# TheRealOrange/icer_compression

Hardware: AMD Instinct MI355X
Metric: Mpixels/s encode (bit-exact), 4096x4096 gray (higher is better)
Workload: dtype int16

## Files before the change

### icer_compression_amd/csrc/coder_core.hpp

```cpp
#pragma once
#include "events.hpp"
#include "icer_tables.hpp"
#include "wave.hpp"

#if defined(ICER_ISA_MARKERS) && !defined(ICER_WAVE_EMU)
#define ICER_STR2(x) #x
#define ICER_STR(x) ICER_STR2(x)
#define ICER_MARK(what) asm volatile("; ICER_MARK " what " line " ICER_STR(__LINE__));
#else
#define ICER_MARK(what)
#endif

#if defined(ICER_WAVE_EMU) && defined(ICER_WAVE_THREADS)
#include <assert.h>
#include <atomic>
#include <thread>
#define ICER_EMU_COUNT(i)
#define ICER_LOAD_CNT(x) __atomic_load_n(&(x), __ATOMIC_ACQUIRE)
#define ICER_POLL_PAUSE(n) std::this_thread::yield()
#define ICER_SET_ABORT2() __atomic_store_n(&s.abort, 2u, __ATOMIC_RELAXED)
#define ICER_FENCE_ACQ() std::atomic_thread_fence(std::memory_order_acquire)
#define ICER_FENCE_REL() std::atomic_thread_fence(std::memory_order_release)
#define ICER_STORE_CNT(x, v) __atomic_store_n(&(x), (v), __ATOMIC_RELEASE)
#define ICER_LANE0
// ... 311 lines not shown
                {                                                                                     \
                    if (PRED) {                                                                       \
                        LV(TOUT) = t0_ + (uint32_t)mbcnt64(m_, lane);                                 \
                        LV(ZOUT) = z0_ + (uint32_t)mbcnt64(zm_, lane);                                \
                    }                                                                                 \
                }                                                                                     \
                FOR_LANES { if ((uint32_t)lane == (C)) { LV(ctot) = t0_ + n_; LV(czer) = z0_ + nz_; } }      \
            } else {                                                                                  \
                const uint32_t kc_ = kRescaleCap - 1 - t0_;   \
                const int lc_ = ffs64(BALLOT((PRED) && (uint32_t)mbcnt64(m_, lane) == kc_));          \
                const uint32_t zc_ = (uint32_t)popc64(zm_ & ((2ull << lc_) - 1ull));                  \
                const uint32_t zat_ = z0_ + zc_;                                                      \
                const uint32_t zr_ = (zat_ > kRescaleCap / 2) ? (zat_ >> 1) : zat_;                   \
                FOR_LANES                                                                             \
                {                                                                                     \
                    if (PRED) {                                                                       \
                        const uint32_t rk_ = (uint32_t)mbcnt64(m_, lane), zb_ = (uint32_t)mbcnt64(zm_, lane); \
                        if (rk_ <= kc_) { LV(TOUT) = t0_ + rk_; LV(ZOUT) = z0_ + zb_; }               \
                        else { LV(TOUT) = kRescaleCap / 2 + (rk_ - kc_ - 1); LV(ZOUT) = zr_ + (zb_ - zc_); } \
                    }                                                                                 \
                }                                                                                     \
                FOR_LANES { if ((uint32_t)lane == (C)) { LV(ctot) = kRescaleCap / 2 + (n_ - kc_ - 1); LV(czer) = zr_ + (nz_ - zc_); } } \
            }                                                                                         \
        }                                                                                             \
    }

ICER_DEV bool flush_stage(CoderShared &s, const UnitArgs &a, bool final_partial)
{
    DECL_LANE;
    const uint32_t bp = s.bitpos;
    const uint32_t first = s.flushed_words;
    uint32_t last = bp >> 5;
    if (final_partial && (bp & 31u)) last++;
    const bool fits = last <= a.cap_words;
    const uint32_t stop = fits ? last : a.cap_words;
    FOR_LANES
    {
        for (uint32_t wi = first + (uint32_t)lane; wi < last; wi += 64) {
            const uint32_t v = s.stage[wi & (kStageWords - 1)];
            if (wi < stop) a.out_words[wi] = v;
            s.stage[wi & (kStageWords - 1)] = 0;
        }
    }
    WAVE_SYNC();
    FOR_LANES
    {
        if (lane == 0) s.flushed_words = last;
    }
    WAVE_SYNC();
    return fits && (bp >> 3) < a.cap_words * 4u;
}

ICER_DEV uint64_t below64(uint32_t x) { return x >= 64u ? ~0ull : ((1ull << x) - 1ull); }
ICER_DEV uint32_t own_bit(uint64_t A, int lane) { return ((lane < 32 ? (uint32_t)A : (uint32_t)(A >> 32)) >> (lane & 31)) & 1u; }
ICER_DEV uint64_t lanes_below(int lane)
{
    const uint32_t lo = lane < 32 ? (1u << (lane & 31)) - 1u : ~0u, hi = lane < 32 ? 0u : (1u << (lane & 31)) - 1u;
    return (uint64_t)lo | ((uint64_t)hi << 32);
}
ICER_DEV uint32_t cnt_lt(uint64_t A1, uint64_t A2, uint32_t pos)
{
    return (uint32_t)(popc64(A1 & below64((pos + 1u) >> 1)) + popc64(A2 & below64(pos >> 1)));
}
ICER_DEV uint32_t cnt_lt_own(uint64_t A1, uint64_t A2, int lane, uint32_t slot)
{
    return (uint32_t)(mbcnt64(A1, lane) + mbcnt64(A2, lane)) + (slot ? own_bit(A1, lane) : 0u);
}
ICER_DEV int last_le(uint64_t A1, uint64_t A2, uint32_t pos)
{
    const uint64_t c1 = A1 & below64((pos >> 1) + 1u), c2 = A2 & below64((pos + 1u) >> 1);
    const int k1 = c1 ? 2 * (63 - clz64(c1)) : -1, k2 = c2 ? 2 * (63 - clz64(c2)) + 1 : -1;
    return k1 > k2 ? k1 : k2;
}
ICER_DEV int last_lt(uint64_t A1, uint64_t A2, uint32_t pos) { return pos == 0u ? -1 : last_le(A1, A2, pos - 1u); }
ICER_DEV int last_lt_own(uint64_t A1, uint64_t A2, int lane, uint32_t slot)
{
    const uint64_t lt = lanes_below(lane);
    const uint64_t c1 = A1 & (slot ? (lt << 1) | 1ull : lt), c2 = A2 & lt;
    const int k1 = c1 ? 2 * (63 - clz64(c1)) : -1, k2 = c2 ? 2 * (63 - clz64(c2)) + 1 : -1;
    return k1 > k2 ? k1 : k2;
}
ICER_DEV int last_le_own(uint64_t A1, uint64_t A2, int lane, uint32_t slot)
{
    const uint64_t lt = lanes_below(lane), le = (lt << 1) | 1ull;
    const uint64_t c1 = A1 & le, c2 = A2 & (slot ? le : lt);
    const int k1 = c1 ? 2 * (63 - clz64(c1)) : -1, k2 = c2 ? 2 * (63 - clz64(c2)) + 1 : -1;
    return k1 > k2 ? k1 : k2;
}
ICER_DEV uint32_t cnt_lt1(uint64_t A1, uint32_t pos) { return (uint32_t)popc64(A1 & below64((pos + 1u) >> 1)); }
ICER_DEV uint32_t cnt_lt_own1(uint64_t A1, int lane, uint32_t slot) { return (uint32_t)mbcnt64(A1, lane) + (slot ? own_bit(A1, lane) : 0u); }
ICER_DEV int last_lt_own1(uint64_t A1, int lane, uint32_t slot)
{
    const uint64_t lt = lanes_below(lane);
    const uint64_t c1 = A1 & (slot ? (lt << 1) | 1ull : lt);
    return c1 ? 2 * (63 - clz64(c1)) : -1;
}
ICER_DEV int last_le_own1(uint64_t A1, int lane)
{
    const uint64_t c1 = A1 & ((lanes_below(lane) << 1) | 1ull);
    return c1 ? 2 * (63 - clz64(c1)) : -1;
}

ICER_DEV uint32_t wave_drain(CoderShared &s, uint32_t limit, uint32_t max_rounds)
{
    DECL_LANE;
    const uint32_t popped0 = s.popped;
    uint32_t head = popped0 & (kRingWords - 1), used = limit - popped0, bitpos = s.bitpos;
    uint32_t npop = 0;
    for (uint32_t round = 0; round < max_rounds; round++) {
        LANEVAR(uint32_t, w); LANEVAR(uint32_t, len); LANEVAR(uint32_t, off);
        FOR_LANES
        {
            LV(w) = (uint32_t)lane < used ? RING_LD((head + (uint32_t)lane) & (kRingWords - 1)) : 0u;
        }
        const uint64_t done = BALLOT((LV(w) & kWordDone) != 0u);
        const uint32_t n = (uint32_t)ffs64(~done);
        if (n == 0) break;
        FOR_LANES
        {
            LV(len) = (uint32_t)lane < n ? ((LV(w) >> 11) & 15u) : 0u;
        }
        const uint64_t L0 = BALLOT(LV(len) & 1u), L1 = BALLOT(LV(len) & 2u), L2 = BALLOT(LV(len) & 4u), L3 = BALLOT(LV(len) & 8u);
        const uint32_t total = (uint32_t)(popc64(L0) + 2 * popc64(L1) + 4 * popc64(L2) + 8 * popc64(L3));
        FOR_LANES
        {
            LV(off) = (uint32_t)(mbcnt64(L0, lane) + 2 * mbcnt64(L1, lane) + 4 * mbcnt64(L2, lane) + 8 * mbcnt64(L3, lane));
        }
        FOR_LANES
        {
            if (LV(len)) {
                const uint32_t p = bitpos + LV(off), wi = (p >> 5) & (kStageWords - 1), sh = p & 31u;
                const uint32_t code = LV(w) & 0x3FFu;
                LDS_OR(s.stage[wi], code << sh);
                if (sh + LV(len) > 32u) LDS_OR(s.stage[(wi + 1) & (kStageWords - 1)], code >> (32u - sh));
            }
        }
        bitpos += total;
        head = (head + n) & (kRingWords - 1);
        used -= n;
        npop += n;
        if (n < 64u) break;
    }
    WAVE_SYNC();
    FOR_LANES
    {
        if (lane == 0) s.bitpos = bitpos;
    }
    ICER_PUBLISH(s.popped, popped0 + npop)
    WAVE_SYNC();
    return npop;
}


struct PixelWave {
    LANEVAR(uint32_t, nb);
    uint32_t fetched = ~0u;
    uint64_t blank = 0;
    uint32_t blank_base = ~0u;
};

#define ICER_BLANK_MASK(J)                                                                             \
    if (((J) & ~63u) != cw.blank_base) {                                                               \
        cw.blank_base = (J) & ~63u;                                                                    \
        cw.blank = BALLOT(cw.blank_base + (uint32_t)lane < nchunks && (uint32_t)a.sig[cw.blank_base + (uint32_t)lane] <= lsb); \
    }
#define ICER_IS_BLANK(J) (((cw.blank >> ((J) & 63u)) & 1ull) != 0ull)

#define ICER_UNPACK_EVENT_BYTE(B, V1, C1, B1, V2, C2, B2)                                              \
    {                                                                                                  \
        const uint32_t b_ = (B), c4_ = b_ & 15u;                                                       \
        V1 = c4_ != kEvNone ? 1u : 0u;                                                                 \
        C1 = c4_ == kEvUncoded ? 31u : c4_;                                                            \
        B1 = (b_ >> 4) & 1u;                                                                           \
        V2 = (c4_ <= 8u && (b_ & 16u)) ? 1u : 0u;        \
        C2 = 12u + ((b_ >> 5) & 3u);                                                                   \
        B2 = (b_ >> 7) & 1u;                                                                           \
    }

ICER_DEV void pixel_wave_run(CoderShared &s, const UnitArgs &a, PixelWave &cw, uint32_t j0, uint32_t j1, uint32_t k, uint32_t npw)
{
    DECL_LANE;
    ICER_TIMERS_DECL
    const uint32_t nchunks = (a.w * a.h + 63u) / 64u;
    const uint32_t lsb = (uint32_t)a.lsb;
    const uint32_t jfirst = j0 + (k + npw - j0 % npw) % npw;
    if (cw.fetched != jfirst && jfirst < nchunks) {
        ICER_BLANK_MASK(jfirst)
        if (!ICER_IS_BLANK(jfirst)) { FOR_LANES { LV(cw.nb) = a.ev[(size_t)jfirst * 64u + (uint32_t)lane]; } }
        cw.fetched = jfirst;
    }

    for (uint32_t j = jfirst; j < j1; j += npw) {
        LANEVAR(uint32_t, valid1); LANEVAR(uint32_t, ctx1); LANEVAR(uint32_t, bit1);
        LANEVAR(uint32_t, valid2); LANEVAR(uint32_t, ctx2); LANEVAR(uint32_t, bit2);
        ICER_BLANK_MASK(j)
        const bool blank = ICER_IS_BLANK(j);
        LANEVAR(uint32_t, eb);
        FOR_LANES { LV(eb) = blank ? 0u : LV(cw.nb); }
        if (j + npw < nchunks) {
            ICER_BLANK_MASK(j + npw)
            if (!ICER_IS_BLANK(j + npw)) { FOR_LANES { LV(cw.nb) = a.ev[(size_t)(j + npw) * 64u + (uint32_t)lane]; } }
        }
        cw.fetched = j + npw;
        FOR_LANES { ICER_UNPACK_EVENT_BYTE(LV(eb), LV(valid1), LV(ctx1), LV(bit1), LV(valid2), LV(ctx2), LV(bit2)) }
        LANEVAR(uint32_t, w1); LANEVAR(uint32_t, w2); LANEVAR(uint32_t, cnw);
#define ICER_MATCH(KEY, V, B0, B1, B2, B3) \
        ((V) & (((KEY)&1u) ? (B0) : ~(B0)) & (((KEY)&2u) ? (B1) : ~(B1)) & (((KEY)&4u) ? (B2) : ~(B2)) & (((KEY)&8u) ? (B3) : ~(B3)))
#ifdef ICER_WAVE_EMU
        assert(blank == (BALLOT(!LV(valid1) || LV(ctx1) != 0u || LV(bit1) != 0u || LV(valid2)) == 0ull));
#endif
        if (blank) {
            FOR_LANES
            {
                LV(w1) = 0x80u | ((uint32_t)lane << 8) | ((uint32_t)lane << 16);
                LV(w2) = 0;
                LV(cnw) = lane == 0 ? (64u | (64u << 8)) : 0u;
            }
        } else {
            const uint64_t V = BALLOT(LV(valid1) && LV(ctx1) != 31u);
            const uint64_t B0 = BALLOT(LV(ctx1) & 1u), B1 = BALLOT(LV(ctx1) & 2u), B2 = BALLOT(LV(ctx1) & 4u), B3 = BALLOT(LV(ctx1) & 8u);
            const uint64_t ZM = BALLOT(LV(bit1) == 0u);
            const uint64_t U = BALLOT(LV(valid2) != 0u);
            const uint64_t C0 = BALLOT((LV(ctx2) - 12u) & 1u), C1 = BALLOT((LV(ctx2) - 12u) & 2u), C2 = BALLOT((LV(ctx2) - 12u) & 4u);
            const uint64_t ZN = BALLOT(LV(bit2) == 0u);
            LANEVAR(uint32_t, om_lo); LANEVAR(uint32_t, om_hi); LANEVAR(uint32_t, g1l); LANEVAR(uint32_t, g1h); LANEVAR(uint32_t, g2l); LANEVAR(uint32_t, g2h);
            LANEVAR(uint32_t, x1); LANEVAR(uint32_t, x2);
            FOR_LANES
            {
                uint64_t m = 0, zs = ZM;
                if (U) {
                    const bool sg = lane >= 12;
                    const uint32_t key = sg ? (uint32_t)lane - 12u : (uint32_t)lane;
                    const uint64_t vv = sg ? U : V, b0 = sg ? C0 : B0, b1 = sg ? C1 : B1, b2 = sg ? C2 : B2, b3 = sg ? 0ull : B3;
                    if (lane <= 16) m = ICER_MATCH(key, vv, b0, b1, b2, b3);
                    zs = sg ? ZN : ZM;
                } else if (lane < 12) m = ICER_MATCH((uint32_t)lane, V, B0, B1, B2, B3);
                LV(om_lo) = (uint32_t)m; LV(om_hi) = (uint32_t)(m >> 32);
                LV(cnw) = (uint32_t)popc64(m) | ((uint32_t)popc64(m & zs) << 8);
                LV(x1) = LV(ctx1) & 31u; LV(x2) = LV(ctx2) & 31u;
                LV(g1l) = 0; LV(g1h) = 0; LV(g2l) = 0; LV(g2h) = 0;
            }
            WAVE_GATHER(g1l, om_lo, x1) WAVE_GATHER(g1h, om_hi, x1)
            if (U) { WAVE_GATHER(g2l, om_lo, x2) WAVE_GATHER(g2h, om_hi, x2) }
            FOR_LANES
            {
                LV(w1) = 0; LV(w2) = 0;
                if (LV(valid1)) {
                    LV(w1) = 0x80u | (LV(bit1) << 5) | LV(ctx1);
                    if (LV(ctx1) != 31u) {
                        const uint64_t m = (uint64_t)LV(g1l) | ((uint64_t)LV(g1h) << 32);
                        LV(w1) |= ((uint32_t)mbcnt64(m, lane) << 8) | ((uint32_t)mbcnt64(m & ZM, lane) << 16);
                    }
                }
                if (LV(valid2)) {
                    LV(w2) = 0x80u | (LV(bit2) << 5) | LV(ctx2);
                    const uint64_t m = (uint64_t)LV(g2l) | ((uint64_t)LV(g2h) << 32);
                    LV(w2) |= ((uint32_t)mbcnt64(m, lane) << 8) | ((uint32_t)mbcnt64(m & ZN, lane) << 16);
                }
            }
        }
#undef ICER_MATCH
        ICER_TICK(0)
        ICER_WAIT_CNT(s.a_done, ad_, j < ad_ + kQueueDepth, ab_, ICER_BP_SLEEP)
        if (ab_) break;
        ICER_TICK(1)
        PixelSlot &o = s.pq[j % kQueueDepth];
        FOR_LANES
        {
            o.e[lane][0] = LV(w1);
            o.e[lane][1] = LV(w2);
            if (lane < 17) o.cn[lane] = (uint16_t)LV(cnw);
            if (lane == 17) o.cn[17] = blank ? 1u : 0u;
        }
        ICER_PUBLISH(s.p_done[k], j + 1u)
    }
    ICER_TIMERS_STORE(a.timers)
}

struct CountWave {
    LANEVAR(uint32_t, czer);
    LANEVAR(uint32_t, ctot);
};

ICER_DEV void count_wave_run(CoderShared &s, const UnitArgs &a, CountWave &cs, uint32_t j0, uint32_t j1, uint32_t npw)
{
    DECL_LANE;
    ICER_TIMERS_DECL
    LANEVAR(uint32_t, czer); LANEVAR(uint32_t, ctot);
    FOR_LANES
    {
        LV(czer) = j0 == 0 ? 2u : LV(cs.czer);
        LV(ctot) = j0 == 0 ? 4u : LV(cs.ctot);
    }
    for (uint32_t j = j0; j < j1; j++) {
        ICER_WAIT_CNT(s.p_done[j % npw], pd_, pd_ > j, ab_, 1)
        if (ab_) break;
        ICER_TICK(2)
        const PixelSlot &in = s.pq[j % kQueueDepth];
        LANEVAR(uint32_t, valid1); LANEVAR(uint32_t, ctx1); LANEVAR(uint32_t, bit1);
        LANEVAR(uint32_t, valid2); LANEVAR(uint32_t, ctx2); LANEVAR(uint32_t, bit2);
        LANEVAR(uint32_t, z1); LANEVAR(uint32_t, t1); LANEVAR(uint32_t, z2); LANEVAR(uint32_t, t2);
        LANEVAR(uint32_t, rk1); LANEVAR(uint32_t, zb1); LANEVAR(uint32_t, rk2); LANEVAR(uint32_t, zb2);
        LANEVAR(uint32_t, cn); LANEVAR(uint32_t, cnz);
        FOR_LANES
        {
            const uint32_t c1 = in.e[lane][0], c2 = in.e[lane][1];
            LV(valid1) = (c1 >> 7) & 1u; LV(ctx1) = c1 & 31u; LV(bit1) = (c1 >> 5) & 1u; LV(rk1) = (c1 >> 8) & 255u; LV(zb1) = (c1 >> 16) & 255u;
            LV(valid2) = (c2 >> 7) & 1u; LV(ctx2) = c2 & 31u; LV(bit2) = (c2 >> 5) & 1u; LV(rk2) = (c2 >> 8) & 255u; LV(zb2) = (c2 >> 16) & 255u;
            const uint32_t w = lane < 17 ? (uint32_t)in.cn[lane] : 0u;
            LV(cn) = w & 255u; LV(cnz) = w >> 8;
            LV(z1) = 1; LV(t1) = 2;
            LV(z2) = 0; LV(t2) = 0;
        }

#ifdef ICER_WAVE_THREADS
        assert(ICER_LOAD_CNT(s.p_done[j % npw]) <= j + kQueueDepth);
#endif
        {
            LANEVAR(uint32_t, t0); LANEVAR(uint32_t, zz0); LANEVAR(uint32_t, idx);
            FOR_LANES { LV(idx) = LV(ctx1) & 15u; }
            WAVE_GATHER(t0, ctot, idx)
            WAVE_GATHER(zz0, czer, idx)
            FOR_LANES
            {
                if (LV(valid1) && LV(ctx1) != 31u) { LV(t1) = LV(t0) + LV(rk1); LV(z1) = LV(zz0) + LV(zb1); }
                LV(idx) = LV(ctx2);
            }
            if (BALLOT(LV(valid2) != 0u)) {
                WAVE_GATHER(t0, ctot, idx)
                WAVE_GATHER(zz0, czer, idx)
            }
            LANEVAR(uint32_t, cross);
            FOR_LANES
            {
                if (LV(valid2)) { LV(t2) = LV(t0) + LV(rk2); LV(z2) = LV(zz0) + LV(zb2); }
                LV(cross) = 0;
                if (lane < 17) {
                    if (LV(ctot) + LV(cn) < kRescaleCap) { LV(ctot) += LV(cn); LV(czer) += LV(cnz); }
                    else LV(cross) = 1;
                }
            }
            for (uint64_t rem = BALLOT(LV(cross) != 0u); rem; rem &= rem - 1ull) {
                const uint32_t c = (uint32_t)ffs64(rem);
                if (c < 12u) ICER_CTX_STEP(c, LV(valid1) && LV(ctx1) == c, LV(bit1) == 0u, z1, t1)
                else ICER_CTX_STEP(c, LV(valid2) && LV(ctx2) == c, LV(bit2) == 0u, z2, t2)
            }
        }
        ICER_TICK(3)

        LANEVAR(uint32_t, ev1); LANEVAR(uint32_t, ev2);
        FOR_LANES
        {
            uint32_t e1 = 0, e2 = 0;
            if (LV(valid1)) {
                uint32_t z = LV(z1), t = LV(t1), b = LV(bit1);
                if (z < (t >> 1)) { z = t - z; b ^= 1u; }
                e1 = 0x80u | (b << 5) | pick_bin(s.tab.binlut, z, t);
            }
            if (LV(valid2)) {
                uint32_t z = LV(z2), t = LV(t2), b = LV(bit2);
                if (z < (t >> 1)) { z = t - z; b ^= 1u; }
                e2 = 0x80u | (b << 5) | pick_bin(s.tab.binlut, z, t);
            }
            LV(ev1) = e1;
            LV(ev2) = e2;
        }
        ICER_TICK(4)
        ICER_WAIT_CNT(s.b_done, bd_, j < bd_ + kQueueDepth, ab2_, ICER_BP_SLEEP)
        if (ab2_) break;
        ICER_TICK(5)
        EventSlot &q = s.eq[j % kQueueDepth];
        FOR_LANES
        {
            q.ev1[lane] = (uint8_t)LV(ev1);
            q.ev2[lane] = (uint8_t)LV(ev2);
            if (lane == 0) q.blank = in.cn[17];
            if (lane < kNumBins) q.cnt[lane] = LV(czer) | (LV(ctot) << 16);
        }
        ICER_PUBLISH(s.a_done, j + 1u)
    }
    FOR_LANES { LV(cs.czer) = LV(czer); LV(cs.ctot) = LV(ctot); }
    ICER_TIMERS_STORE(a.timers)
}

constexpr uint32_t kPrefixRing = 32;
struct PrefixRing {
    uint16_t cn[kPrefixRing][20];
    uint8_t ev[kPrefixRing][64];
};
static_assert(sizeof(PrefixRing) <= sizeof(EventSlot) * kQueueDepth, "the prefix ring lies over the event queue");
ICER_DEV PrefixRing &prefix_ring(CoderShared &s) { return *reinterpret_cast<PrefixRing *>(&s.eq[0]); }

ICER_DEV void pixel_prefix_run(CoderShared &s, const UnitArgs &a, PixelWave &cw, uint32_t j0, uint32_t j1, uint32_t k, uint32_t npw)
{
    DECL_LANE;
    PrefixRing &ring = prefix_ring(s);
    const uint32_t nchunks = (a.w * a.h + 63u) / 64u;
    const uint32_t lsb = (uint32_t)a.lsb;
    const uint32_t jfirst = j0 + (k + npw - j0 % npw) % npw;
    if (cw.fetched != jfirst && jfirst < nchunks) {
        ICER_BLANK_MASK(jfirst)
        if (!ICER_IS_BLANK(jfirst)) { FOR_LANES { LV(cw.nb) = a.ev[(size_t)jfirst * 64u + (uint32_t)lane]; } }
        cw.fetched = jfirst;
    }
    for (uint32_t j = jfirst; j < j1; j += npw) {
        ICER_BLANK_MASK(j)
        const bool blank = ICER_IS_BLANK(j);
        LANEVAR(uint32_t, eb); LANEVAR(uint32_t, cnw);
        FOR_LANES { LV(eb) = blank ? 0u : LV(cw.nb); }
        if (j + npw < nchunks) {
            ICER_BLANK_MASK(j + npw)
            if (!ICER_IS_BLANK(j + npw)) { FOR_LANES { LV(cw.nb) = a.ev[(size_t)(j + npw) * 64u + (uint32_t)lane]; } }
        }
        cw.fetched = j + npw;
        if (blank) {
            FOR_LANES { LV(cnw) = lane == 0 ? (64u | (64u << 8)) : 0u; }
        } else {
            LANEVAR(uint32_t, valid1); LANEVAR(uint32_t, ctx1); LANEVAR(uint32_t, bit1);
            LANEVAR(uint32_t, valid2); LANEVAR(uint32_t, ctx2); LANEVAR(uint32_t, bit2);
            FOR_LANES { ICER_UNPACK_EVENT_BYTE(LV(eb), LV(valid1), LV(ctx1), LV(bit1), LV(valid2), LV(ctx2), LV(bit2)) }
#define ICER_MATCH(KEY, V, B0, B1, B2, B3) \
            ((V) & (((KEY)&1u) ? (B0) : ~(B0)) & (((KEY)&2u) ? (B1) : ~(B1)) & (((KEY)&4u) ? (B2) : ~(B2)) & (((KEY)&8u) ? (B3) : ~(B3)))
            const uint64_t V = BALLOT(LV(valid1) && LV(ctx1) != 31u);
            const uint64_t B0 = BALLOT(LV(ctx1) & 1u), B1 = BALLOT(LV(ctx1) & 2u), B2 = BALLOT(LV(ctx1) & 4u), B3 = BALLOT(LV(ctx1) & 8u);
            const uint64_t ZM = BALLOT(LV(bit1) == 0u);
            const uint64_t U = BALLOT(LV(valid2) != 0u);
            const uint64_t C0 = BALLOT((LV(ctx2) - 12u) & 1u), C1 = BALLOT((LV(ctx2) - 12u) & 2u), C2 = BALLOT((LV(ctx2) - 12u) & 4u);
            const uint64_t ZN = BALLOT(LV(bit2) == 0u);
            FOR_LANES
            {
                const bool sg = lane >= 12;
                const uint32_t key = sg ? (uint32_t)lane - 12u : (uint32_t)lane;
                const uint64_t vv = sg ? U : V, b0 = sg ? C0 : B0, b1 = sg ? C1 : B1, b2 = sg ? C2 : B2, b3 = sg ? 0ull : B3;
                const uint64_t m = lane <= 16 ? ICER_MATCH(key, vv, b0, b1, b2, b3) : 0ull;
                LV(cnw) = (uint32_t)popc64(m) | ((uint32_t)popc64(m & (sg ? ZN : ZM)) << 8);
            }
#undef ICER_MATCH
        }
        ICER_WAIT_CNT(s.a_done, ad_, j < ad_ + kPrefixRing, ab_, 2)
        if (ab_) break;
        FOR_LANES
        {
            if (lane < 17) ring.cn[j % kPrefixRing][lane] = (uint16_t)LV(cnw);
            ring.ev[j % kPrefixRing][lane] = (uint8_t)LV(eb);
        }
        ICER_PUBLISH(s.p_done[k], j + 1u)
    }
}

ICER_DEV uint32_t prefix_frontier(CoderShared &s, uint32_t npw)
{
    DECL_LANE;
    LANEVAR(uint32_t, nxt);
    FOR_LANES
    {
        const uint32_t pd = (uint32_t)lane < npw ? ICER_LOAD_CNT(s.p_done[lane]) : 0u;
        LV(nxt) = (uint32_t)lane < npw ? ~(pd ? pd - 1u + npw : (uint32_t)lane) : 0u;
    }
    uint32_t m;
    WAVE_MAX(m, nxt)
    return ~m;
}

ICER_DEV void count_prefix_run(CoderShared &s, const UnitArgs &a, CountWave &cs, uint32_t j0, uint32_t j1, uint32_t npw)
{
    DECL_LANE;
    (void)a;
    PrefixRing &ring = prefix_ring(s);
    LANEVAR(uint32_t, czer); LANEVAR(uint32_t, ctot);
    FOR_LANES
    {
        LV(czer) = j0 == 0 ? 2u : LV(cs.czer);
        LV(ctot) = j0 == 0 ? 4u : LV(cs.ctot);
    }
    uint32_t avail = j0;
    for (uint32_t j = j0; j < j1; j++) {
        if (j >= avail) {
            avail = prefix_frontier(s, npw);
            if (avail <= j) {
                ICER_PUBLISH(s.a_done, j)
                ICER_WAIT_UNTIL((avail = prefix_frontier(s, npw)) > j || ICER_LOAD_CNT(s.abort))
            }
            if (ICER_LOAD_CNT(s.abort)) break;
            ICER_ACQUIRE()
        }
        LANEVAR(uint32_t, cross);
        FOR_LANES
        {
            const uint32_t w = lane < 17 ? (uint32_t)ring.cn[j % kPrefixRing][lane] : 0u;
            LV(cross) = 0;
            if (lane < 17) {
                if (LV(ctot) + (w & 255u) < kRescaleCap) { LV(ctot) += w & 255u; LV(czer) += w >> 8; }
                else LV(cross) = 1;
            }
        }
        uint64_t rem = BALLOT(LV(cross) != 0u);
        if (rem) {
            LANEVAR(uint32_t, v1); LANEVAR(uint32_t, c1); LANEVAR(uint32_t, b1); LANEVAR(uint32_t, v2); LANEVAR(uint32_t, c2); LANEVAR(uint32_t, b2);
            LANEVAR(uint32_t, zo); LANEVAR(uint32_t, to);
            FOR_LANES
            {
                ICER_UNPACK_EVENT_BYTE((uint32_t)ring.ev[j % kPrefixRing][lane], LV(v1), LV(c1), LV(b1), LV(v2), LV(c2), LV(b2))
                LV(zo) = 0; LV(to) = 0;
            }
            (void)zo; (void)to;
            for (; rem; rem &= rem - 1ull) {
                const uint32_t c = (uint32_t)ffs64(rem);
                if (c < 12u) ICER_CTX_STEP(c, LV(v1) && LV(c1) == c, LV(b1) == 0u, zo, to)
                else ICER_CTX_STEP(c, LV(v2) && LV(c2) == c, LV(b2) == 0u, zo, to)
            }
        }
        if ((j & 7u) == 7u) ICER_PUBLISH(s.a_done, j + 1u)
    }
    ICER_PUBLISH(s.a_done, j1)
    FOR_LANES { LV(cs.czer) = LV(czer); LV(cs.ctot) = LV(ctot); }
}

ICER_DEV void compact_wave_run(CoderShared &s, const UnitArgs &a, uint32_t j0, uint32_t j1)
{
    DECL_LANE;
    ICER_TIMERS_DECL
    for (uint32_t j = j0; j < j1; j++) {
#if !defined(ICER_WAVE_EMU) || defined(ICER_WAVE_THREADS)
        if ((j & 127u) == 127u && quota_already_spent(a)) { ICER_PUBLISH(s.abort, 3u) break; }
#endif
        ICER_WAIT_CNT(s.a_done, ad_, ad_ > j, ab_, 1)
        if (ab_) break;
        ICER_ACQUIRE()
        ICER_TICK(25)
        EventSlot &q = s.eq[j % kQueueDepth];
        LANEVAR(uint32_t, ev1); LANEVAR(uint32_t, ev2);
        FOR_LANES
        {
            LV(ev1) = q.ev1[lane];
            LV(ev2) = q.ev2[lane];
        }
        const uint64_t V1 = BALLOT((LV(ev1) & 0x98u) == 0x80u && (LV(ev1) & 7u)), V2 = BALLOT((LV(ev2) & 0x98u) == 0x80u && (LV(ev2) & 7u));
        if ((V1 | V2) == 0ull) {
            FOR_LANES
            {
                if (lane < 8) q.binn[lane] = 0;
            }
            ICER_PUBLISH(s.c_done, j + 1u)
            ICER_TICK(26)
            continue;
        }
        FOR_LANES
        {
            if (lane < 48) (&q.binbits[0][0])[lane] = 0;
        }
        WAVE_SYNC();
        {
#define ICER_MATCH3(KEY, V, B0, B1, B2) ((V) & (((KEY)&1u) ? (B0) : ~(B0)) & (((KEY)&2u) ? (B1) : ~(B1)) & (((KEY)&4u) ? (B2) : ~(B2)))
            const uint64_t P0 = BALLOT(LV(ev1) & 1u), P1 = BALLOT(LV(ev1) & 2u), P2 = BALLOT(LV(ev1) & 4u);
            LANEVAR(uint32_t, oa_lo); LANEVAR(uint32_t, oa_hi); LANEVAR(uint32_t, ob_lo); LANEVAR(uint32_t, ob_hi);
            LANEVAR(uint32_t, i1); LANEVAR(uint32_t, i2);
            LANEVAR(uint32_t, a1l); LANEVAR(uint32_t, a1h); LANEVAR(uint32_t, b1l); LANEVAR(uint32_t, b1h);
            LANEVAR(uint32_t, a2l); LANEVAR(uint32_t, a2h); LANEVAR(uint32_t, b2l); LANEVAR(uint32_t, b2h);
            if (V2) {
                const uint64_t Q0 = BALLOT(LV(ev2) & 1u), Q1 = BALLOT(LV(ev2) & 2u), Q2 = BALLOT(LV(ev2) & 4u);
                FOR_LANES
                {
                    const uint64_t ma = ICER_MATCH3((uint32_t)lane & 7u, V1, P0, P1, P2), mb = ICER_MATCH3((uint32_t)lane & 7u, V2, Q0, Q1, Q2);
                    LV(oa_lo) = (uint32_t)ma; LV(oa_hi) = (uint32_t)(ma >> 32); LV(ob_lo) = (uint32_t)mb; LV(ob_hi) = (uint32_t)(mb >> 32);
                    if (lane < 8) q.binn[lane] = (uint8_t)(popc64(ma) + popc64(mb));
                    LV(i1) = LV(ev1) & 7u; LV(i2) = LV(ev2) & 7u;
                }
                WAVE_GATHER(a1l, oa_lo, i1) WAVE_GATHER(a1h, oa_hi, i1) WAVE_GATHER(b1l, ob_lo, i1) WAVE_GATHER(b1h, ob_hi, i1)
                WAVE_GATHER(a2l, oa_lo, i2) WAVE_GATHER(a2h, oa_hi, i2) WAVE_GATHER(b2l, ob_lo, i2) WAVE_GATHER(b2h, ob_hi, i2)
            } else {
                FOR_LANES
                {
                    const uint64_t ma = ICER_MATCH3((uint32_t)lane & 7u, V1, P0, P1, P2);
                    LV(oa_lo) = (uint32_t)ma; LV(oa_hi) = (uint32_t)(ma >> 32);
                    if (lane < 8) q.binn[lane] = (uint8_t)popc64(ma);
                    LV(i1) = LV(ev1) & 7u;
                    LV(b1l) = 0; LV(b1h) = 0; LV(a2l) = 0; LV(a2h) = 0; LV(b2l) = 0; LV(b2h) = 0;
                }
                WAVE_GATHER(a1l, oa_lo, i1) WAVE_GATHER(a1h, oa_hi, i1)
            }
            FOR_LANES
            {
                if ((V1 >> lane) & 1ull) {
                    const uint32_t b = LV(ev1) & 7u;
                    const uint64_t m1 = (uint64_t)LV(a1l) | ((uint64_t)LV(a1h) << 32), m2 = (uint64_t)LV(b1l) | ((uint64_t)LV(b1h) << 32);
                    const uint32_t r = (uint32_t)(mbcnt64(m1, lane) + mbcnt64(m2, lane));
                    q.rk1[lane] = (uint8_t)r;
                    q.binseq[b][r] = (uint8_t)(2u * (uint32_t)lane);
                    if (LV(ev1) & 0x20u) LDS_OR(q.binbits[b][(r + 8u) >> 5], 1u << ((r + 8u) & 31u));
                }
                if ((V2 >> lane) & 1ull) {
                    const uint32_t b = LV(ev2) & 7u;
                    const uint64_t m1 = (uint64_t)LV(a2l) | ((uint64_t)LV(a2h) << 32), m2 = (uint64_t)LV(b2l) | ((uint64_t)LV(b2h) << 32);
                    const uint32_t r = (uint32_t)(mbcnt64(m1, lane) + (int)((m1 >> lane) & 1ull) + mbcnt64(m2, lane));
                    q.rk2[lane] = (uint8_t)r;
                    q.binseq[b][r] = (uint8_t)(2u * (uint32_t)lane + 1u);
                    if (LV(ev2) & 0x20u) LDS_OR(q.binbits[b][(r + 8u) >> 5], 1u << ((r + 8u) & 31u));
                }
            }
// ... 1005 lines not shown
```

### icer_compression_amd/csrc/kernels.hpp

```cpp
#pragma once
#include <hip/hip_runtime.h>

#include "assemble_core.hpp"
#include "assemble_ladder.hpp"
#include "coder_core.hpp"
#include "coder_wg.hpp"
#include "coder_wg_small.hpp"
#include "dwt_tile.hpp"
#include "events.hpp"
#include "plan.hpp"

namespace icer {

__global__ void __launch_bounds__(kTileThreads)
dwt_tile_kernel(DwtStageArgs a, size_t src_plane, size_t coef_plane, size_t ll_plane, int *__restrict__ ovf)
{
    __shared__ union { DwtTileShared gen; DwtFastShared fast; } u;
    a.src += blockIdx.z * src_plane;
    a.coef += blockIdx.z * coef_plane;
    a.ll += blockIdx.z * ll_plane;
    const int tx = blockIdx.x, ty = blockIdx.y, t = threadIdx.x;
    if (dwt_tile_is_interior(a, tx, ty)) {
        bool o = dwt_fast_rows_step1(u.fast, a, tx, ty, t);
        __syncthreads();
// ... 43 lines not shown
    mean_ovf[p] = m > (sample_bits == 8 ? 127 : 32767) ? 1 : 0;
}

__global__ void __launch_bounds__(256)
finalize_ll_kernel(uint16_t *__restrict__ coef, size_t plane, uint32_t w, uint32_t llw, uint32_t llh,
                   const uint16_t *__restrict__ means, const int *__restrict__ frame_skip, int channels, int sample_bits)
{
    const uint32_t c = blockIdx.x * 64 + (threadIdx.x & 63), r = blockIdx.y * 4 + (threadIdx.x >> 6);
    if (c >= llw || r >= llh) return;
    if (frame_skip[blockIdx.z / channels]) return;
    uint16_t *q = coef + blockIdx.z * plane + (size_t)r * w + c;
    const int16_t v = (int16_t)((int16_t)*q - (int16_t)means[blockIdx.z]);
    *q = (uint16_t)to_coder_word(v, sample_bits);
}

struct SplitLaunch {
    const SubDesc *subs = nullptr;
    const uint32_t *launch = nullptr;
    uint32_t n_subs = 0;
    uint32_t entries = 0;
    Snapshot *snaps = nullptr;
    uint32_t *snap_valid = nullptr;
    SubRecord *recs = nullptr;
};

constexpr uint8_t kRoutePipeline = 0, kRouteWindows = 1, kRouteNoSplit = 2;

template <int WAVES, int OCC, int LDS_PAD>
__global__ void __launch_bounds__(64 * WAVES, OCC)
code_units_kernel(const uint16_t *__restrict__ coef, size_t plane, uint32_t img_w, uint32_t img_h, int channels,
                  const UnitDesc *__restrict__ units, const uint32_t *__restrict__ work_order, uint32_t n_units,
                  const CoderTables *__restrict__ tables, const uint16_t *__restrict__ means,
                  const int *__restrict__ frame_skip, uint8_t *__restrict__ slots,
                  size_t slot_frame_stride, uint32_t *__restrict__ unit_bits, uint64_t *__restrict__ timers,
                  uint32_t *__restrict__ done_bytes, uint64_t early_quota, const uint8_t *__restrict__ route, SplitLaunch sp, uint32_t n_frames_1d,
                  const uint8_t *__restrict__ ev, size_t ev_frame_stride, const uint8_t *__restrict__ sig, size_t sig_frame_stride,
                  uint32_t fail_inject)
{
    __shared__ CoderShared s;
    if constexpr (LDS_PAD > 0) {
        __shared__ uint32_t lds_pad[LDS_PAD / 4];
        if (early_quota == ~0ull) lds_pad[threadIdx.x] = 1u;
    }
    uint32_t frame = blockIdx.y, lpos = blockIdx.x;
    if (gridDim.y == 1u && n_frames_1d > 1u) {
        position_major(blockIdx.x, n_units + sp.n_subs, n_frames_1d, &frame, &lpos);
        if (frame >= n_frames_1d) return;
    }
    const uint32_t entry = sp.n_subs ? sp.launch[lpos] : (work_order ? work_order[lpos] : lpos);
    const bool sub_block = sp.n_subs != 0u && (entry >> 31) != 0u;
    const SubDesc sd = sub_block ? sp.subs[entry & 0x7FFFFFFFu] : SubDesc{};
    const uint32_t ui = sub_block ? sd.unit : entry;
    const uint8_t rt = route ? route[(size_t)frame * n_units + ui] : kRoutePipeline;
    if (rt == kRouteWindows) return;
    if (sub_block && rt != kRoutePipeline) return;
#ifdef ICER_PHASE_TIMERS
    uint64_t *trace = (timers && frame == 0 && lpos < (uint32_t)kTraceUnits) ? timers + 9 * 32 + 4 * lpos : nullptr;
    if (trace && threadIdx.x == 0) {
        trace[0] = wall_clock64();
        trace[2] = (uint64_t)__builtin_amdgcn_s_getreg((31 << 11) | 4) | ((uint64_t)__builtin_amdgcn_s_getreg((3 << 11) | 20) << 32);
        trace[3] = entry;
    }
    if (timers && frame == 0 && lpos == 0 && (threadIdx.x & 63) == 0)
        timers[9 * 32 + 4 * kTraceUnits + (threadIdx.x >> 6)] = (uint64_t)__builtin_amdgcn_s_getreg((31 << 11) | 4);
#endif
    const uint32_t wave = (uint32_t)__builtin_amdgcn_readfirstlane((int)(threadIdx.x >> 6));
    if (frame_skip[frame]) {
        if (threadIdx.x == 0 && !sub_block) unit_bits[(size_t)frame * n_units + ui] = 0;
        return;
    }
    const UnitDesc u = units[ui];
    const bool injected = fail_inject == ((frame << 20) | ui);
    if (early_quota) {
        UnitArgs pa;
        pa.done_bytes = done_bytes + (size_t)frame * n_units; pa.prio_index = ui; pa.early_quota = early_quota;
        __shared__ int skip_unit;
        if (wave == 0) {
            const bool spent = quota_already_spent(pa);
            if (threadIdx.x == 0) skip_unit = spent ? 1 : 0;
        }
        __syncthreads();
        if (skip_unit) {
            if (threadIdx.x == 0) unit_bits[(size_t)frame * n_units + ui] = 0;
            return;
        }
    }
    switch (u.prio) {
    case 3: __builtin_amdgcn_s_setprio(3); break;
    case 2: __builtin_amdgcn_s_setprio(2); break;
    case 1: __builtin_amdgcn_s_setprio(1); break;
    default: break;
    }
    {
        const uint32_t *src = reinterpret_cast<const uint32_t *>(tables);
        uint32_t *dst = reinterpret_cast<uint32_t *>(&s.tab);
        for (uint32_t i = threadIdx.x; i < sizeof(CoderTables) / 4; i += 64 * WAVES) dst[i] = src[i];
    }
    constexpr uint32_t kWalker = 0, kPixel = 1, kGolomb = 2, kMerge = 3, kCompact = 4, kCount = 5, kRecords = 6, kDrain = 7;
    constexpr uint32_t kGolombState = 8, kPixel2 = 9, kGolomb2 = 10;
    static_assert(WAVES == kUnitWavesSmall || WAVES == kUnitWavesLarge, "two shapes of a workgroup");
    constexpr bool large = WAVES == kUnitWavesLarge;
    constexpr uint32_t npw = large ? 2u : 1u, ngw = large ? 2u : 0u;
    if (wave == 0) unit_state_init(s);
    if (threadIdx.x == 64) s.nchunks = (u.w * u.h + 63u) / 64u;
    if (wave == kMerge) build_crc_table(s);

    uint32_t *slot_words = reinterpret_cast<uint32_t *>(slots + (size_t)frame * slot_frame_stride + u.slot_off);
    UnitArgs a;
    a.seg = coef + ((size_t)frame * channels + u.chan) * plane + (size_t)u.y0 * img_w + u.x0;
    a.stride = img_w;
    a.ev = ev + (size_t)frame * ev_frame_stride + ev_offset(u.lsb, sig_frame_stride, u.sig_off, 0u);
    a.sig = sig + (size_t)frame * sig_frame_stride + u.sig_off;
    a.w = u.w; a.h = u.h;
    a.subband = (int)u.subband; a.lsb = (int)u.lsb;
    a.out_words = slot_words + kHeaderBytes / 4;
    a.cap_words = u.cap_words;
    __shared__ SubLayout layout;
    const bool split = sp.n_subs != 0u && u.n_sub > 1u && rt == kRoutePipeline;
    if (split) {
        if (threadIdx.x == 0) {
            layout.n_sub = u.n_sub;
            layout.index = sub_block ? sd.index : 0u;
            for (uint32_t i = 0; i <= u.n_sub; i++) layout.first[i] = sub_first_chunk((u.w * u.h + 63u) / 64u, u.n_sub, i);
            const size_t e = (size_t)frame * sp.entries + u.sub_entry;
            layout.snaps = sp.snaps + e * kMaxSnaps;
            layout.snap_valid = sp.snap_valid + e * kMaxSnaps;
            layout.rec = sp.recs + e;
        }
        a.sub = &layout;
        if (sub_block) {
            a.out_words = reinterpret_cast<uint32_t *>(slots + (size_t)frame * slot_frame_stride + sd.slot_off);
            a.cap_words = sd.cap_words;
        }
    }
    a.done_bytes = early_quota ? done_bytes + (size_t)frame * n_units : nullptr;
    a.prio_index = ui;
    a.early_quota = early_quota;
    a.timers = (timers && u.level == 1) ? timers + u.lsb * 32 : nullptr;
    const uint32_t nchunks = (u.w * u.h + 63u) / 64u;
    __syncthreads();

    uint32_t j0 = 0;
    CountWave cs;
    if (split && sub_block) {
        j0 = layout.first[layout.index];
        constexpr uint32_t npw1 = (uint32_t)(WAVES - 1) < kMaxPixelWaves ? (uint32_t)(WAVES - 1) : kMaxPixelWaves;
        const uint32_t k = wave < kCount ? wave : wave - 1u;
        if (wave == kCount) count_prefix_run(s, a, cs, 0, j0, npw1);
        else if (k < npw1) {
            PixelWave pw;
            pixel_prefix_run(s, a, pw, 0, j0, k, npw1);
        }
        __syncthreads();
        const uint32_t ab1 = s.abort;
        __syncthreads();
        if (ab1) {
            if (wave == kMerge) {
                SubRecord &r = layout.rec[layout.index];
                if ((threadIdx.x & 63) == 0) { r.end_chunk = j0; r.end_bits = kUnitFailed; r.match_sub = 0; r.match_snap = 0; }
                const int lane = (int)(threadIdx.x & 63);
                ICER_AGENT_PUBLISH(&r.done, 1u)
            }
            return;
        }
        if (wave == 0) unit_state_init(s, j0);
        __syncthreads();
    }

    if (wave == kPixel || wave == kPixel2) {
        PixelWave pw;
        pixel_wave_run(s, a, pw, j0, nchunks, wave == kPixel ? 0u : 1u, npw);
    } else if (wave == kCount) {
        count_wave_run(s, a, cs, j0, nchunks, npw);
    } else if (wave == kWalker) {
        WalkWave ww;
        walk_wave_init(s, ww, j0);
        walk_wave_run(s, a, ww, nchunks, ~0u);
    } else if (wave == kGolomb || wave == kGolomb2) {
        GolombWave gw;
        golomb_wave_init(gw, j0);
        golomb_wave_run(s, a, gw, nchunks, ~0u, wave == kGolomb ? 0u : 1u, ngw);
    } else if (wave == kGolombState) {
        GolombWave gw;
        golomb_wave_init(gw, j0);
        golomb_state_run(s, a, gw, nchunks, ~0u);
    } else if (wave == kRecords) {
        RecordsWave rw;
        rw.next = j0;
        records_wave_run(s, a, rw, ~0u);
    } else if (wave == kDrain) {
        drain_wave_run(s, a, ~0u);
    } else if (wave == kCompact) {
        compact_wave_run(s, a, j0, nchunks);
    } else if (split) {
        const uint32_t how = merge_wave_run(s, a, j0, nchunks);
        if (how != kMergeMatched) {
            uint32_t bits = how == kMergeDone ? merge_wave_finish(s, a) : kUnitTooBig;
            if (s.abort == 2u || injected) bits = kUnitFailed;
            SubRecord &r = layout.rec[layout.index];
            if ((threadIdx.x & 63) == 0) { r.end_chunk = nchunks; r.end_bits = bits; r.match_sub = 0; r.match_snap = 0; }
            const int lane = (int)(threadIdx.x & 63);
            ICER_AGENT_PUBLISH(&r.done, 1u)
        }
#ifdef ICER_PHASE_TIMERS
        if (trace && (threadIdx.x & 63) == 0) { trace[1] = wall_clock64(); trace[3] |= (uint64_t)(how == kMergeMatched ? layout.rec[layout.index].end_chunk : nchunks) << 32; }
#endif
    } else {
        uint32_t bits = merge_wave_run(s, a, 0, nchunks) ? merge_wave_finish(s, a) : kUnitTooBig;
        if (s.abort == 2u || injected) {
            bits = kUnitFailed;
            if (injected && (threadIdx.x & 63) == 0) s.abort_site = 0xFFFFu | (0xFFu << 16);
            if ((threadIdx.x & 63) == 0 && u.cap_words >= kFailWords) {
                uint32_t *dbg = slot_words + kHeaderBytes / 4;
                dbg[0] = kFailMagic; dbg[1] = s.abort_site; dbg[2] = nchunks; dbg[3] = s.p_done[0]; dbg[4] = s.a_done;
                dbg[5] = s.c_done; dbg[6] = s.b_done; dbg[7] = s.alloc; dbg[8] = s.popped; dbg[9] = s.hold_seq;
                dbg[10] = s.hold_ack; dbg[11] = s.exact_seq; dbg[12] = s.last_exact; dbg[13] = s.bitpos;
                dbg[14] = s.flushed_words; dbg[15] = s.drain_exit;
            }
        }
        if (s.abort == 3u) bits = 0;
        if (bits != kUnitTooBig && bits != kUnitFailed) {
            __threadfence();
            FinishArgs f;
            f.slot_words = slot_words;
            f.bits = bits;
            f.mean = means[(size_t)frame * channels + u.chan];
            f.level = u.level; f.subband = u.subband; f.seg = u.seg; f.lsb = u.lsb; f.chan = u.chan;
            f.image_w = img_w; f.image_h = img_h;
            finish_unit_wave(s, f);
        }
        if ((threadIdx.x & 63) == 0) {
            unit_bits[(size_t)frame * n_units + ui] = bits;
            if (early_quota && s.abort != 3u) {
                const uint32_t d = bits == kUnitTooBig ? (u.cap_is_bound ? 0u : ~0u) : bits == kUnitFailed ? 0u : kHeaderBytes + ((bits + 7u) >> 3);
                __hip_atomic_store(&done_bytes[(size_t)frame * n_units + ui], d, __ATOMIC_RELAXED, __HIP_MEMORY_SCOPE_AGENT);
            }
        }
#ifdef ICER_PHASE_TIMERS
        if (trace && (threadIdx.x & 63) == 0) trace[1] = wall_clock64();
#endif
    }
}

constexpr uint32_t kSpliceWaves = 4;
__global__ void __launch_bounds__(64 * kSpliceWaves)
splice_units_kernel(const UnitDesc *__restrict__ units, uint32_t n_units, const CoderTables *__restrict__ tables,
                    const uint16_t *__restrict__ means, const int *__restrict__ frame_skip, int channels, uint32_t img_w, uint32_t img_h,
                    uint8_t *__restrict__ slots, size_t slot_frame_stride, uint32_t *__restrict__ unit_bits,
                    const uint8_t *__restrict__ route, SplitLaunch sp)
{
    struct SpliceShared { uint32_t crc_tab[256]; struct { uint32_t x2n[32]; } tab; uint32_t parts[kSpliceWaves]; };
    __shared__ SpliceShared s;
    const uint32_t frame = blockIdx.y, ui = blockIdx.x;
    const UnitDesc u = units[ui];
    if (u.n_sub <= 1u || frame_skip[frame]) return;
    if (route && route[(size_t)frame * n_units + ui] != kRoutePipeline) return;
    build_crc_table(s);
    if (threadIdx.x < 32) s.tab.x2n[threadIdx.x] = tables->x2n[threadIdx.x];
    __syncthreads();
    uint8_t *fs = slots + (size_t)frame * slot_frame_stride;
    uint32_t *slot_words = reinterpret_cast<uint32_t *>(fs + u.slot_off);
    uint32_t *words[kMaxSubs];
    words[0] = slot_words + kHeaderBytes / 4;
    for (uint32_t i = 1; i < u.n_sub; i++) words[i] = reinterpret_cast<uint32_t *>(fs + sp.subs[u.sub_first + i - 1u].slot_off);
    const size_t e = (size_t)frame * sp.entries + u.sub_entry;
    __builtin_amdgcn_fence(__ATOMIC_ACQUIRE, "agent");
    const uint32_t wv = threadIdx.x >> 6;
    const uint32_t bits = splice_unit_wave(u.n_sub, sp.recs + e, sp.snaps + e * kMaxSnaps, words, u.cap_words, wv, kSpliceWaves);
    if (bits != kUnitTooBig && bits != kUnitFailed) {
        __threadfence();
        FinishArgs f;
        f.slot_words = slot_words;
        f.bits = bits;
        f.mean = means[(size_t)frame * channels + u.chan];
        f.level = u.level; f.subband = u.subband; f.seg = u.seg; f.lsb = u.lsb; f.chan = u.chan;
        f.image_w = img_w; f.image_h = img_h;
        __syncthreads();
        finish_unit_wave(s, f, wv, kSpliceWaves, s.parts);
    }
    if (threadIdx.x == 0) unit_bits[(size_t)frame * n_units + ui] = bits;
}

__global__ void __launch_bounds__(256)
family_events_kernel(const uint16_t *__restrict__ coef, size_t plane, uint32_t img_w, int channels,
                     const UnitDesc *__restrict__ units, const uint32_t *__restrict__ blocks, const int *__restrict__ frame_skip,
                     uint8_t *__restrict__ sig, size_t sig_frame_stride, uint32_t *__restrict__ hist, uint32_t n_families,
                     uint8_t *__restrict__ ev, size_t ev_frame_stride, uint32_t n_planes)
{
    __shared__ uint8_t ctx_tab[48];
    const UnitDesc u = units[blocks[2u * blockIdx.x]];
    const uint32_t frame = blockIdx.y, nchunks = (u.w * u.h + 63u) / 64u, first = blocks[2u * blockIdx.x + 1u] * 64u;
    if (frame_skip[frame]) return;
    const bool is_hl = u.subband == kHL, is_hh = u.subband == kHH;
    if (ev) {
        if (threadIdx.x < 45u) ctx_tab[threadIdx.x] = (uint8_t)ev_ctx_entry(is_hh, threadIdx.x);
        __syncthreads();
    }
    const uint16_t *seg = coef + ((size_t)frame * channels + u.chan) * plane + (size_t)u.y0 * img_w + u.x0;
    uint8_t *out = sig + (size_t)frame * sig_frame_stride + u.sig_off;
    uint8_t *evf = ev ? ev + (size_t)frame * ev_frame_stride : nullptr;
    const uint32_t wave = threadIdx.x >> 6, lane = threadIdx.x & 63u;
    const uint32_t sw = u.w, sh = u.h, npix = sw * sh;
    uint32_t j = first + wave * 16u;
    uint32_t np = j * 64u + lane;
    uint32_t r = np / sw, c = np - r * sw;
    uint32_t mine = 0;
// ... 316 lines not shown
```

Measured before the change: 3385.

## Deepen pixel prefix event prefetch to an 8-slot register ring and prefetch sig blocks

The pixel prefix wave now keeps an 8-entry per-lane register queue of event chunks fetched ahead, instead of one chunk prefetched one step ahead. This hides global memory latency on the sequential prefix scan. It also prefetches the next 64-chunk significance block, so the blank-mask ballot does not wait on a fresh load. The cost is higher register pressure from the unrolled queue, plus fetches of event data even for blank chunks. A debug phase timer gated behind a macro is added.

```diff
diff --git a/icer_compression_amd/csrc/coder_core.hpp b/icer_compression_amd/csrc/coder_core.hpp
--- a/icer_compression_amd/csrc/coder_core.hpp
+++ b/icer_compression_amd/csrc/coder_core.hpp
@@ -487,11 +487,15 @@
 }
 
 
+constexpr uint32_t kPrefixAhead = 8;
 struct PixelWave {
     LANEVAR(uint32_t, nb);
     uint32_t fetched = ~0u;
     uint64_t blank = 0;
     uint32_t blank_base = ~0u;
+    LANEVAR(uint32_t, pq[kPrefixAhead]);
+    LANEVAR(uint32_t, nsig);
+    uint32_t sig_base = ~0u;
 };
 
 #define ICER_BLANK_MASK(J)                                                                             \
@@ -733,20 +737,35 @@
     const uint32_t nchunks = (a.w * a.h + 63u) / 64u;
     const uint32_t lsb = (uint32_t)a.lsb;
     const uint32_t jfirst = j0 + (k + npw - j0 % npw) % npw;
-    if (cw.fetched != jfirst && jfirst < nchunks) {
-        ICER_BLANK_MASK(jfirst)
-        if (!ICER_IS_BLANK(jfirst)) { FOR_LANES { LV(cw.nb) = a.ev[(size_t)jfirst * 64u + (uint32_t)lane]; } }
+    uint32_t q0 = (jfirst / npw) % kPrefixAhead;
+    if (cw.fetched != jfirst) {
+#if !defined(ICER_WAVE_EMU)
+#pragma unroll
+#endif
+        for (uint32_t q = 0; q < kPrefixAhead; q++) {
+            const uint32_t jq = jfirst + ((q + kPrefixAhead - q0) % kPrefixAhead) * npw;
+            if (jq < nchunks) { FOR_LANES { LV(cw.pq[q]) = a.ev[(size_t)jq * 64u + (uint32_t)lane]; } }
+        }
         cw.fetched = jfirst;
     }
-    for (uint32_t j = jfirst; j < j1; j += npw) {
-        ICER_BLANK_MASK(j)
+    for (uint32_t j = jfirst; j < j1; q0 = 0u) {
+#if !defined(ICER_WAVE_EMU)
+#pragma unroll
+#endif
+      for (uint32_t q = 0; q < kPrefixAhead; q++) {
+        if (q < q0 || j >= j1) continue;
+        if ((j & ~63u) != cw.blank_base) {
+            const uint32_t base = j & ~63u;
+            if (cw.sig_base != base) { FOR_LANES { LV(cw.nsig) = base + (uint32_t)lane < nchunks ? (uint32_t)a.sig[base + (uint32_t)lane] : 255u; } }
+            cw.blank = BALLOT(base + (uint32_t)lane < nchunks && LV(cw.nsig) <= lsb);
+            cw.blank_base = base;
+            cw.sig_base = base + 64u;
+            FOR_LANES { LV(cw.nsig) = base + 64u + (uint32_t)lane < nchunks ? (uint32_t)a.sig[base + 64u + (uint32_t)lane] : 255u; }
+        }
         const bool blank = ICER_IS_BLANK(j);
         LANEVAR(uint32_t, eb); LANEVAR(uint32_t, cnw);
-        FOR_LANES { LV(eb) = blank ? 0u : LV(cw.nb); }
-        if (j + npw < nchunks) {
-            ICER_BLANK_MASK(j + npw)
-            if (!ICER_IS_BLANK(j + npw)) { FOR_LANES { LV(cw.nb) = a.ev[(size_t)(j + npw) * 64u + (uint32_t)lane]; } }
-        }
+        FOR_LANES { LV(eb) = blank ? 0u : LV(cw.pq[q]); }
+        if (j + kPrefixAhead * npw < nchunks) { FOR_LANES { LV(cw.pq[q]) = a.ev[(size_t)(j + kPrefixAhead * npw) * 64u + (uint32_t)lane]; } }
         cw.fetched = j + npw;
         if (blank) {
             FOR_LANES { LV(cnw) = lane == 0 ? (64u | (64u << 8)) : 0u; }
@@ -773,13 +792,15 @@
 #undef ICER_MATCH
         }
         ICER_WAIT_CNT(s.a_done, ad_, j < ad_ + kPrefixRing, ab_, 2)
-        if (ab_) break;
+        if (ab_) return;
         FOR_LANES
         {
             if (lane < 17) ring.cn[j % kPrefixRing][lane] = (uint16_t)LV(cnw);
             ring.ev[j % kPrefixRing][lane] = (uint8_t)LV(eb);
         }
         ICER_PUBLISH(s.p_done[k], j + 1u)
+        j += npw;
+      }
     }
 }
 
diff --git a/icer_compression_amd/csrc/kernels.hpp b/icer_compression_amd/csrc/kernels.hpp
--- a/icer_compression_amd/csrc/kernels.hpp
+++ b/icer_compression_amd/csrc/kernels.hpp
@@ -219,6 +219,9 @@
             pixel_prefix_run(s, a, pw, 0, j0, k, npw1);
         }
         __syncthreads();
+#ifdef ICER_PHASE_TIMERS
+        if (trace && threadIdx.x == 0) trace[2] |= ((uint64_t)sd.index << 36) | (((wall_clock64() - trace[0]) & 0xFFFFFFull) << 40);
+#endif
         const uint32_t ab1 = s.abort;
         __syncthreads();
         if (ab1) {
```

After: 3388, median of 4. No clear change (+0.1%).
